# CC834/Heterogeneous-OpenCL-Image-Processing-Engine

Hardware: AMD Instinct MI355X
Metric: images_per_sec (higher is better)
Workload: dtype u8

## Files before the change

heterogeneous-opencl-image-processing-engine_amd/__init__.py:

```python
from __future__ import annotations

import ctypes as C
import os
import re
import subprocess

PKG_DIR = os.path.dirname(os.path.abspath(__file__))
ROOT = os.path.dirname(PKG_DIR)
CSRC = os.path.join(PKG_DIR, "csrc")
APPS = os.path.join(PKG_DIR, "apps")
LIB_PATH = os.path.join(PKG_DIR, "libmi_blur.so")
HEADER = os.path.join(ROOT, "include", "mi_blur.h")
HIPCC = os.environ.get("HIPCC", "/opt/rocm/bin/hipcc")
os.environ.setdefault("HIP_FORCE_DEV_KERNARG", "0")
ARCH = "gfx950"

DEVICE_CPU = -1
VARIANT_AUTO, VARIANT_GENERIC, VARIANT_TILED, VARIANT_STREAM, VARIANT_DIRECT = 0, 1, 2, 3, 4
OK, ERR_INVALID, ERR_NO_DEVICE, ERR_NOMEM, ERR_STATE, ERR_UNSUPPORTED = 0, -1, -2, -3, -4, -5
UNIQUE_ID_BYTES = 128
SEP_MAX_RADIUS = 16
MEDIAN_MAX_RADIUS = 7
MORPH_MAX_RADIUS = 16
MORPH_ERODE, MORPH_DILATE, MORPH_GRADIENT = 0, 1, 2
# ... 431 lines not shown
        "mi_blur_cpu_run_warp": (i, [u8p, u8p, i, i, i, i, C.POINTER(Warp), i]),
        "mi_blur_ctx_set_warp": (i, [vp, C.POINTER(Warp)]),
        "mi_blur_warp_perspective_coord": (i, [C.POINTER(WarpPerspective), i, i, C.POINTER(C.c_int64), C.POINTER(C.c_int64), C.POINTER(i), C.POINTER(i)]),
        "mi_blur_warp_perspective_quad": (i, [C.POINTER(C.c_double), C.POINTER(C.c_double), C.POINTER(C.c_double)]),
        "mi_blur_warp_perspective_set_matrix": (i, [C.POINTER(WarpPerspective), C.POINTER(C.c_double), i]),
        "mi_blur_enqueue_warp_perspective": (i, [u8p, u8p, i, i, i, i, C.POINTER(WarpPerspective), vp]),
        "mi_blur_cpu_run_warp_perspective": (i, [u8p, u8p, i, i, i, i, C.POINTER(WarpPerspective), i]),
        "mi_blur_ctx_set_warp_perspective": (i, [vp, C.POINTER(WarpPerspective)]),
        "mi_blur_remap_coord": (i, [C.POINTER(Remap), i, i, C.c_int32, C.c_int32, C.POINTER(i), C.POINTER(i), C.POINTER(i), C.POINTER(i)]),
        "mi_blur_remap_from_float": (i, [vp, vp, C.c_size_t, vp]),
        "mi_blur_remap_undistort": (i, [C.POINTER(C.c_double), C.POINTER(C.c_double), C.POINTER(C.c_double), i, i, vp]),
        "mi_blur_remap_plan": (i, [vp, i, i, i, C.POINTER(Remap), C.POINTER(RemapTiles)]),
        "mi_blur_enqueue_remap": (i, [u8p, u8p, i, i, i, i, C.POINTER(Remap), vp, vp]),
        "mi_blur_cpu_run_remap": (i, [u8p, u8p, i, i, i, i, C.POINTER(Remap), vp, i]),
        "mi_blur_ctx_set_remap": (i, [vp, C.POINTER(Remap), vp]),
        "mi_blur_conv_preset": (i, [i, C.POINTER(Conv)]),
        "mi_blur_enqueue_conv": (i, [u8p, u8p, i, i, i, i, C.POINTER(Conv), vp]),
        "mi_blur_enqueue_conv_band": (i, [u8p, u8p, i, i, i, i, i, C.POINTER(Conv), vp]),
        "mi_blur_cpu_run_conv": (i, [u8p, u8p, i, i, i, i, C.POINTER(Conv), i]),
        "mi_blur_ctx_set_conv": (i, [vp, C.POINTER(Conv)]),
        "mi_blur_fill_synthetic": (None, [u8p, i, i, i, i, i, i]),
        "mi_blur_fnv1a64": (C.c_uint64, [u8p, C.c_size_t]),
        "mi_blur_debug_zc_trace": (i, [vp, C.POINTER(C.c_uint64), i, C.POINTER(i), C.POINTER(C.c_uint)]),
        "mi_blur_debug_xcd_times": (i, [C.POINTER(C.c_uint64), C.POINTER(C.c_uint64), i]),
        "mi_blur_debug_xcd_raw": (i, [C.POINTER(C.c_uint64), C.c_size_t, C.c_size_t]),
        "mi_blur_a1_partition": (None, [i, i, C.c_float, C.POINTER(i), C.POINTER(i)]),
        "mi_blur_shard_range": (None, [C.c_longlong, i, i, C.POINTER(C.c_longlong), C.POINTER(C.c_longlong)]),
        "mi_blur_a2_split": (None, [i, C.c_float, i, C.POINTER(A2Geometry)]),
        "mi_blur_band_of": (None, [i, i, i, i, C.POINTER(Band)]),
        "mi_blur_comm_unique_id": (i, [vp]),
        "mi_blur_comm_init_rank": (i, [C.POINTER(vp), i, i, vp]),
        "mi_blur_comm_init_all": (i, [C.POINTER(vp), i, C.POINTER(i)]),
        "mi_blur_comm_init_p2p": (i, [C.POINTER(vp), i, C.POINTER(i)]),
        "mi_blur_comm_init_pull": (i, [C.POINTER(vp), i, C.POINTER(i)]),
        "mi_blur_comm_destroy": (None, [vp]),
        "mi_blur_comm_info": (i, [vp, C.POINTER(i), C.POINTER(i), C.POINTER(i)]),
        "mi_blur_halo_exchange": (i, [vp, u8p, i, i, i, i, vp]),
        "mi_blur_peer_export": (i, [vp, vp, C.POINTER(C.c_uint64)]),
        "mi_blur_peer_open": (i, [vp, C.c_uint64, C.POINTER(vp)]),
        "mi_blur_peer_close": (i, [vp, C.c_uint64]),
        "mi_blur_halo_pull": (i, [u8p, u8p, u8p, i, i, i, i, vp]),
        "mi_blur_enqueue_band_peer": (i, [u8p, u8p, i, i, i, i, i, i, u8p, u8p, vp]),
        "mi_blur_halo_exchange_all": (i, [C.POINTER(vp), i, C.POINTER(vp), i, i, C.POINTER(i), i, C.POINTER(vp)]),
    }
    for name, (res, args) in sig.items():
        fn = getattr(L, name)
        fn.restype, fn.argtypes = res, args
# ... 1069 lines not shown
```

heterogeneous-opencl-image-processing-engine_amd/csrc/blur_kernels.hip:

```cpp
#include "kernel_common.h"

#include <math.h>
#include <stdlib.h>
#include <string.h>
#include <mutex>
#include <algorithm>

namespace mi_blur {

__device__ __forceinline__ u16x2 as_pk(uint32_t x) { return __builtin_bit_cast(u16x2, x); }
__device__ __forceinline__ uint32_t as_u32(u16x2 x) { return __builtin_bit_cast(uint32_t, x); }

constexpr uint32_t EVEN_MASK = 0x00ff00ffu;
__device__ __forceinline__ uint32_t even_of(uint32_t x) { return x & EVEN_MASK; }
__device__ __forceinline__ uint32_t odd_of(uint32_t x) { return __builtin_amdgcn_perm(0u, x, 0x0c030c01u); }
__device__ __forceinline__ uint32_t mad6(uint32_t c, uint32_t t) { return as_u32(as_pk(c) * (unsigned short)6 + as_pk(t)); }

constexpr uint32_t sel_left(int C, int q)
{
    uint32_t s = 0;
    for (int j = 0; j < 4; j++) {
        int p = -4 * q + j;
        int idx = ((p % C) + C) % C;
        s |= (uint32_t)idx << (8 * j);
// ... 123 lines not shown
    }
    uint32_t Ew[8], Ow[8];
#pragma unroll
    for (int j = 0; j < 8; j++) { Ew[j] = even_of(w[j]); Ow[j] = odd_of(w[j]); }
    h[0] = hsum<C, R, 0, 0>(Ew, Ow); h[1] = hsum<C, R, 0, 1>(Ew, Ow);
    h[2] = hsum<C, R, 0, 2>(Ew, Ow); h[3] = hsum<C, R, 0, 3>(Ew, Ow);
    h[4] = hsum<C, R, 1, 0>(Ew, Ow); h[5] = hsum<C, R, 1, 1>(Ew, Ow);
    h[6] = hsum<C, R, 1, 2>(Ew, Ow); h[7] = hsum<C, R, 1, 3>(Ew, Ow);
}

struct TiledParams {
    const uint8_t *in;
    uint8_t *out;
    long long in_stride, out_stride;
    int pitch, cpr;
    int H, y0, y1;
    int ncols, nstrips;
    int TH, ntiles_y, ngroups;
    unsigned nblocks;
    int xcd;
    int debug_copy;
    unsigned long long *xcd_times;
    int tail;
};

struct __attribute__((packed, aligned(1))) Unaligned16 { u32x4 v; };
struct __attribute__((packed, aligned(1))) Unaligned8 { u32x2 v; };
struct __attribute__((packed, aligned(1))) Unaligned4 { uint32_t v; };
struct __attribute__((packed, aligned(1))) Unaligned2 { uint16_t v; };

__device__ __forceinline__ void store16_write_through(uint8_t *q, u32x4 v);
__device__ __forceinline__ void store_chunk_ragged_wt(uint8_t *q, u32x4 v, int n);
template <bool WT = false>
__device__ __forceinline__ void store_chunk_ragged(uint8_t *q, u32x4 v, int n)
{
    if constexpr (WT) { store_chunk_ragged_wt(q, v, n); return; }
    if (n >= 16) { reinterpret_cast<Unaligned16 *>(q)->v = v; return; }
    if (n & 8) { u32x2 t; t.x = v.x; t.y = v.y; reinterpret_cast<Unaligned8 *>(q)->v = t; q += 8; v.x = v.z; v.y = v.w; }
    if (n & 4) { reinterpret_cast<Unaligned4 *>(q)->v = v.x; q += 4; v.x = v.y; }
    if (n & 2) { reinterpret_cast<Unaligned2 *>(q)->v = (uint16_t)v.x; q += 2; v.x >>= 16; }
    if (n & 1) *q = (uint8_t)v.x;
}

__device__ __forceinline__ void store16_write_through(uint8_t *q, u32x4 v)
{
    asm volatile("global_store_dwordx4 %0, %1, off sc1\n\ts_nop 1" ::"v"(q), "v"(v) : "memory");
}

__device__ __forceinline__ void store_chunk_ragged_wt(uint8_t *q, u32x4 v, int n)
{
    if (n >= 16) { store16_write_through(q, v); return; }
    if (n & 8) {
        u32x2 t; t.x = v.x; t.y = v.y;
        asm volatile("global_store_dwordx2 %0, %1, off sc1" ::"v"(q), "v"(t) : "memory");
        q += 8; v.x = v.z; v.y = v.w;
    }
    if (n & 4) { asm volatile("global_store_dword %0, %1, off sc1" ::"v"(q), "v"(v.x) : "memory"); q += 4; v.x = v.y; }
    if (n & 2) { asm volatile("global_store_short %0, %1, off sc1" ::"v"(q), "v"(v.x) : "memory"); q += 2; v.x >>= 16; }
    if (n & 1) asm volatile("global_store_byte %0, %1, off sc1" ::"v"(q), "v"(v.x) : "memory");
}

struct NoHook { __device__ __forceinline__ void operator()() const {} };

template <int C, int R, int RPG, bool DMA, bool SHFL, bool RAG, bool WT = false, int X = rowpass_default<R>, typename Hook = NoHook>
__device__ __forceinline__ void tiled_tile(const TiledParams &p, unsigned L, Hook after_staging = Hook{})
{
    extern __shared__ __attribute__((aligned(16))) uint8_t lds[];
    const int t = threadIdx.x, NT = blockDim.x;
    const int strip = (int)(L % (unsigned)p.nstrips);
    const unsigned t2 = L / (unsigned)p.nstrips;
    const int ty = (int)(t2 % (unsigned)p.ntiles_y);
    const int img = (int)(t2 / (unsigned)p.ntiles_y);

    const int ty0 = p.y0 + ty * p.TH;
    const int rows_out = min(p.TH, p.y1 - ty0);
    const int x0c = strip * p.ncols;
    const int nc = min(p.ncols, p.cpr - x0c);
    const int cpr2 = nc + 2;
    const int nrows = rows_out + 2 * R;
    const uint8_t *img_in = p.in + (long long)img * p.in_stride;

    {
        const int lane = t & 63, wv = t >> 6, nwaves = NT >> 6;
        const int rpi = 64 / cpr2;
        const int lr = lane / cpr2, cc = lane - lr * cpr2;
        const bool dead_halo = (cc == 0 && x0c == 0) || (cc == cpr2 - 1 && x0c + nc == p.cpr);
        const bool act = lr < rpi && !dead_halo;
        const unsigned col_off = (unsigned)min(max(x0c + cc - 1, 0), p.cpr - 1) * 16u;
        for (int u = wv; u * rpi < nrows; u += nwaves) {
            const int row = u * rpi + lr;
            if (act && row < nrows) {
                const int sr = min(max(ty0 - R + row, 0), p.H - 1);
                const uint8_t *g = img_in + ((unsigned)sr * (unsigned)p.pitch + col_off);
                if constexpr (RAG) {
                    const uint8_t *rowp = img_in + (size_t)sr * (size_t)p.pitch;
                    uint8_t *dst = lds + (size_t)(u * rpi * cpr2 + lane) * 16u;
                    if (x0c + cc - 1 == p.cpr - 1) {
                        const u32x4 v = reinterpret_cast<const Unaligned16 *>(rowp + p.pitch - 16)->v;
                        reinterpret_cast<Unaligned16 *>(dst - (16 - p.tail))->v = v;
                        const int len = (16 - p.tail) + (cc == cpr2 - 1 ? 0 : 8);
                        uint8_t *pd = dst + p.tail;
                        const uint32_t fill[6] = {clamp_right<C, 0>(v.z, v.w), clamp_right<C, 1>(v.z, v.w), clamp_right<C, 2>(v.z, v.w),
                                                  clamp_right<C, 3>(v.z, v.w), clamp_right<C, 4>(v.z, v.w), clamp_right<C, 5>(v.z, v.w)};
#pragma unroll
                        for (int q = 0; q < 6; q++) {
                            if (4 * q + 4 <= len) reinterpret_cast<Unaligned4 *>(pd + 4 * q)->v = fill[q];
                            else if (4 * q < len)
                                for (int b = 0; b < len - 4 * q; b++) pd[4 * q + b] = (uint8_t)(fill[q] >> (8 * b));
                        }
                    } else if constexpr (DMA) {
                        uint8_t *base = lds + (size_t)(u * rpi * cpr2) * 16u;
                        __builtin_amdgcn_global_load_lds(
// ... 55 lines not shown
            if constexpr (R == 1) {
                const uint32_t se = (((hw[(r + 1) % WIN][i] << 1) + hw[r % WIN][i]) + hw[(r + 2) % WIN][i]) << 4;
                const uint32_t so = (((hw[(r + 1) % WIN][4 + i] << 1) + hw[r % WIN][4 + i]) + hw[(r + 2) % WIN][4 + i]) << 4;
                o[i] = __builtin_amdgcn_perm(so, se, 0x07030501u);
            } else {
                const uint32_t se = mad6(hw[(r + 2) % WIN][i],
                                         ((hw[(r + 1) % WIN][i] + hw[(r + 3) % WIN][i]) << 2) +
                                             (hw[r % WIN][i] + hw[(r + 4) % WIN][i]));
                const uint32_t so = mad6(hw[(r + 2) % WIN][4 + i],
                                         ((hw[(r + 1) % WIN][4 + i] + hw[(r + 3) % WIN][4 + i]) << 2) +
                                             (hw[r % WIN][4 + i] + hw[(r + 4) % WIN][4 + i]));
                o[i] = __builtin_amdgcn_perm(so, se, 0x07030501u);
            }
        }
        if (r0 + r < rows_out) {
            u32x4 v; v.x = o[0]; v.y = o[1]; v.z = o[2]; v.w = o[3];
            if constexpr (RAG) store_chunk_ragged<WT>(op + (size_t)r * (size_t)p.pitch, v, (x0c + col) == p.cpr - 1 ? p.tail : 16);
            else if constexpr (WT) store16_write_through(op + (size_t)r * (size_t)p.pitch, v);
            else *reinterpret_cast<u32x4 *>(op + (size_t)r * (size_t)p.pitch) = v;
        }
    }
}

constexpr unsigned XCD_DEBUG_SLOTS = 1u << 20;
__device__ __forceinline__ void xcd_time_mark(unsigned long long *t, unsigned long long t0)
{
    if (threadIdx.x == 0 && blockIdx.x < XCD_DEBUG_SLOTS) {
        unsigned id;
        asm volatile("s_getreg_b32 %0, hwreg(HW_REG_XCC_ID)" : "=s"(id));
        t[2u * blockIdx.x] = ((unsigned long long)__builtin_amdgcn_s_memrealtime() << 4) | (id & 7u);
        t[2u * blockIdx.x + 1] = t0;
    }
}

template <int C, int R, int RPG, bool DMA, bool SHFL = false, bool RAG = false>
__global__ __launch_bounds__(256) void blur_tiled_kernel(const TiledParams p)
{
    const unsigned long long t0 = p.xcd_times ? __builtin_amdgcn_s_memrealtime() : 0ull;
    tiled_tile<C, R, RPG, DMA, SHFL, RAG>(p, xcd_map(blockIdx.x, p.nblocks, p.xcd));
    if (p.xcd_times) xcd_time_mark(p.xcd_times, t0);
}

template <int C, int R, int RPG>
__global__ __launch_bounds__(256) void blur_tiled_loop_kernel(const TiledParams p)
{
    for (unsigned L = blockIdx.x; L < p.nblocks; L += gridDim.x) {
// ... 98 lines not shown
        const unsigned want = min(tiles_per_batch, total_blocks - first) * per_block;
        unsigned v = 0;
        for (unsigned k = lane; k < kcount; k += 64u) v += __hip_atomic_load(&count[kcount * n + k], __ATOMIC_RELAXED, __HIP_MEMORY_SCOPE_AGENT);
        v += __shfl_xor(v, 1); v += __shfl_xor(v, 2); v += __shfl_xor(v, 4); v += __shfl_xor(v, 8); v += __shfl_xor(v, 16); v += __shfl_xor(v, 32);
        v = __builtin_amdgcn_readfirstlane(v);
        if ((int)(v - want) >= 0) {
            n++;
            continue;
        }
        if (lane == 0) {
            const unsigned long long cur = ((unsigned long long)pass_seq << 32) | n;
            if (__hip_atomic_load(host_word, __ATOMIC_RELAXED, __HIP_MEMORY_SCOPE_SYSTEM) != cur)
                __hip_atomic_store(host_word, cur, __ATOMIC_RELEASE, __HIP_MEMORY_SCOPE_SYSTEM);
        }
        if (wall_clock64() - t0 > ZC_HARD_TICKS) return;
        __builtin_amdgcn_s_sleep(2);
    }
    if (lane == 0) __hip_atomic_store(host_word, ((unsigned long long)pass_seq << 32) | n, __ATOMIC_RELEASE, __HIP_MEMORY_SCOPE_SYSTEM);
}

static_assert(sizeof(TiledParams) <= ZC_PARAM_WORDS * 4 && sizeof(TiledParams) % 4 == 0, "TiledParams must fit a ZcBatch");
static_assert(sizeof(ZcBatch) / 4 <= 64, "the poller copies a descriptor with one wave-instruction");

template <int C, int R, int RPG, bool RAG>
__global__ __launch_bounds__(256) void blur_server_kernel(ZcHostCtl *ctl, ZcDevCtl *dev, unsigned seq, unsigned budget, unsigned idle_ticks,
                                                          unsigned long long *trace, int fixed_share)
{
    const unsigned NW = gridDim.x - 1;
    const unsigned first = dev->next[seq & 1u];

    if (blockIdx.x == NW) {
        const unsigned lane = threadIdx.x;
        if (lane >= 64) return;
        __shared__ unsigned s_ntiles[ZC_RING];
        unsigned g = dev->gnext[seq & 1u];
        if (lane == 0) {
            __hip_atomic_store(&dev->ticket, g, __ATOMIC_RELAXED, __HIP_MEMORY_SCOPE_AGENT);
            __hip_atomic_store(&dev->start_seq, seq + 1u, __ATOMIC_RELEASE, __HIP_MEMORY_SCOPE_AGENT);
        }
        unsigned k = first, c = first;
        const unsigned limit = first + budget;
        bool stopping = false;
        unsigned long long t_idle = wall_clock64();
        for (;;) {
            if (!stopping) {
                unsigned tail = 0;
                if (lane == 0) tail = __hip_atomic_load(&ctl->tail, __ATOMIC_ACQUIRE, __HIP_MEMORY_SCOPE_SYSTEM);
                tail = __builtin_amdgcn_readfirstlane(tail);
                const unsigned target = (int)(tail - limit) > 0 ? limit : tail;
                const bool progressed = (int)(target - k) > 0;
// ... 75 lines not shown
        }
        s_ctl[0] = ok;
    }
    __syncthreads();
    if (!s_ctl[0]) return;
    __syncthreads();
    union { TiledParams p; unsigned words[sizeof(TiledParams) / 4]; } u;
    unsigned k = first, have = 0u, tile_first = 0u, n_tiles = 0u;
    unsigned pending = ~0u;
    auto count_pending = [&]() {
        if (pending != ~0u && threadIdx.x == 0) {
            __builtin_amdgcn_fence(__ATOMIC_RELEASE, "");
            __hip_atomic_fetch_add(&dev->tiles_done[pending], 1u, __ATOMIC_RELEASE, __HIP_MEMORY_SCOPE_AGENT);
        }
        pending = ~0u;
    };
    auto flush_pending = [&]() {
        if (pending != ~0u) {
            asm volatile("s_waitcnt vmcnt(0)" ::: "memory");
            __syncthreads();
            count_pending();
        }
    };
    if (threadIdx.x == 0)
        s_ctl[1] = fixed_share ? dev->gnext[seq & 1u] + w : __hip_atomic_fetch_add(&dev->ticket, 1u, __ATOMIC_RELAXED, __HIP_MEMORY_SCOPE_AGENT);
    __syncthreads();
    unsigned t = s_ctl[1];
    unsigned long long *tr = nullptr;
    for (unsigned it = 0;; it++) {
        for (;;) {
            if (!have) {
                auto look = [&]() -> unsigned {
                    const unsigned a = __hip_atomic_load(&dev->avail, __ATOMIC_ACQUIRE, __HIP_MEMORY_SCOPE_AGENT);
                    if ((int)(a - k) > 0) return 1u;
                    if (__hip_atomic_load(&dev->stop_seq, __ATOMIC_ACQUIRE, __HIP_MEMORY_SCOPE_AGENT) == seq + 1u &&
                        (int)(__hip_atomic_load(&dev->stop_at, __ATOMIC_RELAXED, __HIP_MEMORY_SCOPE_AGENT) - k) <= 0) return 0u;
                    return 2u;
                };
                if (threadIdx.x == 0) s_ctl[0] = look();
                __syncthreads();
                unsigned go = s_ctl[0];
                __syncthreads();
                if (go != 1u) {
                    flush_pending();
                    if (go == 2u) {
                        if (threadIdx.x == 0) {
                            unsigned g2;
                            const unsigned long long t_w = wall_clock64();
                            while ((g2 = look()) == 2u) {
                                if (wall_clock64() - t_w > ZC_HARD_TICKS) { g2 = 0u; __hip_atomic_store(&ctl->error, 3u, __ATOMIC_RELEASE, __HIP_MEMORY_SCOPE_SYSTEM); break; }
// ... 4 lines not shown
                        __syncthreads();
                        go = s_ctl[0];
                        __syncthreads();
                    }
                    if (!go) return;
                }
                if (threadIdx.x < sizeof(ZcBatch) / 4)
                    s_words[threadIdx.x] = __hip_atomic_load(reinterpret_cast<unsigned *>(&dev->batch[k % ZC_RING]) + threadIdx.x, __ATOMIC_RELAXED,
                                                             __HIP_MEMORY_SCOPE_AGENT);
                __syncthreads();
#pragma unroll
                for (unsigned i = 0; i < sizeof(TiledParams) / 4; i++) u.words[i] = __builtin_amdgcn_readfirstlane(s_words[i]);
                tile_first = __builtin_amdgcn_readfirstlane(s_words[ZC_PARAM_WORDS]);
                n_tiles = __builtin_amdgcn_readfirstlane(s_words[ZC_PARAM_WORDS + 1]);
                have = 1u;
                __builtin_amdgcn_fence(__ATOMIC_ACQUIRE, "");
                __syncthreads();
            }
            if ((int)(t - (tile_first + n_tiles)) >= 0) { k++; have = 0u; continue; }
            break;
        }
        tr = (trace && k < ZC_TRACE_BATCHES && threadIdx.x == 0) ? trace + ((size_t)k * NW + w) * 5u : nullptr;
        if (tr) { if (tr[0] == 0) tr[0] = wall_clock64(); tr[1] += 1; }
        if (threadIdx.x == 0)
            s_ctl[2u + (it & 1u)] = fixed_share ? t + NW : __hip_atomic_fetch_add(&dev->ticket, 1u, __ATOMIC_RELAXED, __HIP_MEMORY_SCOPE_AGENT);
        const unsigned long long t_a = trace ? wall_clock64() : 0ull;
        tiled_tile<C, R, RPG, true, false, RAG, false, rowpass_default<R>>(u.p, t - tile_first, count_pending);
        pending = k % ZC_RING;
        __syncthreads();
        if (tr) { tr[2] += wall_clock64() - t_a; tr[3] = wall_clock64(); }
        t = s_ctl[2u + (it & 1u)];
    }
}

constexpr int STREAM_P = 6;
constexpr int STREAM_D = 8;
constexpr int STREAM_ROWB = 32 + 64 * 16;

struct StreamParams {
    const uint8_t *in;
    uint8_t *out;
    long long in_stride, out_stride;
    long long total;
    long long total_images;
    int pitch, cpr;
    int H, y0, y1;
    int BH, nbands;
    unsigned nblocks;
    int xcd;
    int updown;
};

struct StreamLane { unsigned col, band; long long img; };
__device__ __forceinline__ StreamLane stream_decode(unsigned f, const StreamParams &p)
// ... 431 lines not shown
            f.nextra = ntail + (unsigned)((long long)ntail * std::max(10, tun.fused_tail_blocks) / 100);
            g_last_kernel = "blur_fused_tail_kernel";
            const dim3 tgrid(f.nstatic + f.nextra);
            if (fused->gate && tun.fused_overlap > 0 && !ragged) {
                const long long ahead = nblocks * tun.fused_overlap / 1000;
                f.gate = fused->gate; f.gate_seq = fused->seq;
                f.gate_block = (unsigned)std::min<long long>(std::max<long long>(nblocks - ahead, 0), (long long)tgrid.x - 1);
            }
            if (p.xcd_times && tgrid.x <= 65536u) p.xcd_times += 2ull * 65536ull * (fused->seq & 15u);
            return dispatch<1, 2>(R, [&](auto Rc) { return launch_fused_r<Rc>(d, p, f, tgrid, block, lds, rpg, ragged); });
        }
        if (ragged) {
            if (!fused->tail_ctr) return MI_BLUR_ERR_UNSUPPORTED;
            f.tail_ctr = fused->tail_ctr; f.ntail = 0; f.nstatic = (unsigned)nblocks; f.nextra = 0;
            g_last_kernel = "blur_fused_tail_kernel";
        }
        return dispatch<1, 2>(R, [&](auto Rc) { return launch_fused_r<Rc>(d, p, f, grid, block, lds, rpg, ragged); });
    }
    return dispatch<1, 2>(R, [&](auto Rc) {
        return launch_tiled_r<Rc>(d, p, grid, block, lds, rpg, tun.stage_dma != 0, ragged, tun.row_shuffle != 0, tun.experiment);
    });
}

int zc_fill_batch(const LaunchDesc &d, ZcGeometry *geo, ZcBatch *b, unsigned *n_tiles)
{
    if (!geo || !b || !d.in || !d.out || d.n_images <= 0) return MI_BLUR_ERR_INVALID;
    Tunables tun = tunables();
    const bool aligned = tiled_eligible(d.in, d.out, d.width, d.channels) && !(d.in_stride % 16) && !(d.out_stride % 16);
    const long long pitch_b = (long long)d.width * d.channels;
    const bool dense = (!d.in_stride || d.in_stride == pitch_b * d.band_rows) && (!d.out_stride || d.out_stride == pitch_b * (d.y1 - d.y0));
    const bool ragged = !aligned && tun.ragged && ragged_eligible(d.width, d.channels) && dense;
    if (!aligned && !ragged) return MI_BLUR_ERR_UNSUPPORTED;
    tun.debug_copy = 0; tun.debug_xcd_times = 0; tun.xcd_remap = 0;
    TiledParams p{};
    unsigned threads = 0;
    size_t lds = 0;
    const int rpg = tiled_geometry(d, tun, ragged, false, 4, p, &threads, &lds);
    if (rpg < 0) return rpg;
    if (geo->threads == 0) { geo->threads = threads; geo->lds = lds; geo->rpg = rpg; geo->channels = d.channels; geo->radius = d.filter->radius; geo->ragged = ragged ? 1 : 0; }
    else if (geo->threads != threads || geo->lds != lds || geo->rpg != rpg || geo->channels != d.channels || geo->radius != d.filter->radius ||
             geo->ragged != (ragged ? 1 : 0))
        return MI_BLUR_ERR_UNSUPPORTED;
    memset(b->params, 0, sizeof b->params);
    memcpy(b->params, &p, sizeof p);
    if (n_tiles) *n_tiles = p.nblocks;
    return MI_BLUR_OK;
}

int zc_launch_server(const ZcGeometry &geo, ZcHostCtl *ctl, ZcDevCtl *dev, unsigned seq, unsigned n_workers, unsigned budget,
                     unsigned idle_ticks, hipStream_t stream, unsigned long long *trace, int fixed_share)
{
    if (!ctl || !dev || n_workers == 0 || geo.threads == 0 || geo.rpg != 4) return MI_BLUR_ERR_INVALID;
    g_last_kernel = "blur_server_kernel";
    const dim3 grid(n_workers + 1), block(geo.threads);
    return dispatch<0, 1>(geo.ragged, [&](auto RAG) {
        return dispatch<1, 2, 3, 4>(geo.channels, [&](auto C) {
            return dispatch<1, 2>(geo.radius, [&](auto R) {
                return do_launch(blur_server_kernel<C, R, 4, RAG != 0>, grid, block, geo.lds, stream, ctl, dev, seq, budget, idle_ticks, trace, fixed_share);
            });
        });
    });
}

int launch_fused_watch(const unsigned *count, unsigned n_batches, unsigned tiles_per_batch, unsigned total_blocks, unsigned per_block,
                       unsigned long long *host_word, unsigned pass_seq, hipStream_t stream, unsigned counters_per_batch)
{
    if (!count || !host_word || n_batches == 0 || tiles_per_batch == 0 || counters_per_batch < 8 || (counters_per_batch & (counters_per_batch - 1))) return MI_BLUR_ERR_INVALID;
    return do_launch(fused_watch_kernel, dim3(1), dim3(64), 0, stream, count, n_batches, tiles_per_batch, total_blocks, per_block, host_word, pass_seq, counters_per_batch);
}

int launch_fused_gate(const unsigned *gate, unsigned want, hipStream_t stream)
{
    if (!gate) return MI_BLUR_ERR_INVALID;
    return do_launch(fused_gate_kernel, dim3(1), dim3(64), 0, stream, gate, want);
}

int launch_fused(const LaunchDesc &d, const FusedDesc &f)
{
    if (!d.in || !d.out || d.in == d.out || (!f.count && !f.geometry_only) || f.batch_images <= 0) return MI_BLUR_ERR_INVALID;
    if (!d.filter || d.filter->kind != FilterKind::BOX) return MI_BLUR_ERR_INVALID;
    if (d.width <= 0 || d.band_rows <= 0 || d.n_images <= 0 || (d.filter->radius != 1 && d.filter->radius != 2)) return MI_BLUR_ERR_INVALID;
    if (d.y0 != 0 || d.y1 != d.band_rows || d.in_stride || d.out_stride) return MI_BLUR_ERR_INVALID;
// ... 155 lines not shown
```

heterogeneous-opencl-image-processing-engine_amd/csrc/blur_launch.h:

```cpp
#pragma once
#include <hip/hip_runtime.h>
#include <stdint.h>

#include "filter.h"

namespace mi_blur {

struct LaunchDesc {
    const Filter *filter;
    const uint8_t *in;
    uint8_t *out;
    int width, band_rows, channels;
    int n_images;
    int y0, y1;
    long long in_stride, out_stride;
    int concurrent;
    int max_blocks;
    int variant;
    const uint8_t *halo_top, *halo_bottom;
    hipStream_t stream;
    hipEvent_t start, stop;
};

int launch(const LaunchDesc &d);
// ... 55 lines not shown
    unsigned pad[6];
};
struct ZcHostCtl {
    unsigned tail;
    unsigned quit;
    unsigned servers_done;
    unsigned error;
    unsigned pad0[12];
    unsigned done[ZC_RING];
    unsigned long long t_begin[ZC_RING], t_end[ZC_RING];
    ZcBatch batch[ZC_RING];
};
struct ZcDevCtl {
    unsigned next[2];
    unsigned gnext[2];
    unsigned start_seq;
    unsigned avail;
    unsigned stop_seq, stop_at, stop_tile;
    unsigned ticket;
    unsigned pad[6];
    unsigned tiles_done[ZC_RING];
    ZcBatch batch[ZC_RING];
};
struct ZcGeometry { unsigned threads; size_t lds; int rpg; int channels, radius, ragged; };
int zc_fill_batch(const LaunchDesc &d, ZcGeometry *geo, ZcBatch *b, unsigned *n_tiles);
int zc_launch_server(const ZcGeometry &geo, ZcHostCtl *ctl, ZcDevCtl *dev, unsigned seq, unsigned n_workers, unsigned budget,
                     unsigned idle_ticks, hipStream_t stream, unsigned long long *trace = nullptr, int fixed_share = 0);

const char *last_kernel();

bool tiled_eligible(const void *in, const void *out, int width, int channels);

struct Tunables {
    int stage_dma; int rpg; int xcd_remap; int debug_copy; int row_shuffle; int prefer_stream; int stream_bh; int zero_copy; int ragged;
    int fused_release;
    int experiment;
    int xcd_run;
    int zero_copy_streams;
    int zero_copy_blocks;
    int stream_updown;
    int prefer_direct;
    int direct_bh;
    int debug_xcd_times;
    int fused_window;
    int fused_tail;
    int fused_adds_per_word;
    int fused_tail_blocks;
    int fused_overlap;
    int zero_copy_server;
    int zero_copy_server_min_kb;
    int staged_server;
    int zero_copy_workers;
    int zero_copy_idle_us;
    int zero_copy_budget;
    int zero_copy_tickets;
    int resident_place_trials;
    int zero_copy_spin;
    int zero_copy_trace;
    int zero_copy_debug_base;
    int zero_copy_events;
    int integral_band;
    int box_bytes;
    int dist_band;
    int dist_chunk_log2;
};
enum class KnobKind { FLAG, RANGE, ONE_OF };
struct Knob { const char *key; int Tunables::*field; KnobKind kind; int lo, hi, def; const char *env; };
constexpr int knob_bits(int a, int b, int c, int d) { return 1 << a | 1 << b | 1 << c | 1 << d; }
static constexpr Knob KNOBS[] = {
    {"stage_dma", &Tunables::stage_dma, KnobKind::FLAG, 0, 1, 1, "MI_BLUR_STAGE"},
    {"rows_per_thread", &Tunables::rpg, KnobKind::ONE_OF, knob_bits(0, 4, 8, 16), 0, 0, "MI_BLUR_RPG"},
    {"xcd_remap", &Tunables::xcd_remap, KnobKind::FLAG, 0, 1, 1, "MI_BLUR_XCD"},
    {"debug_copy", &Tunables::debug_copy, KnobKind::FLAG, 0, 1, 0, nullptr},
    {"row_shuffle", &Tunables::row_shuffle, KnobKind::FLAG, 0, 1, 0, nullptr},
    {"prefer_stream", &Tunables::prefer_stream, KnobKind::FLAG, 0, 1, 0, nullptr},
    {"zero_copy", &Tunables::zero_copy, KnobKind::FLAG, 0, 1, 1, nullptr},
    {"ragged_tiled", &Tunables::ragged, KnobKind::FLAG, 0, 1, 1, nullptr},
    {"stream_band_rows", &Tunables::stream_bh, KnobKind::RANGE, 0, 4096, 0, nullptr},
    {"fused_release", &Tunables::fused_release, KnobKind::FLAG, 0, 1, 0, nullptr},
    {"experiment", &Tunables::experiment, KnobKind::FLAG, 0, 1, 0, nullptr},
    {"stream_updown", &Tunables::stream_updown, KnobKind::FLAG, 0, 1, 1, nullptr},
    {"zero_copy_streams", &Tunables::zero_copy_streams, KnobKind::RANGE, 1, 8, 4, nullptr},
    {"zero_copy_blocks", &Tunables::zero_copy_blocks, KnobKind::RANGE, 0, 1 << 20, 24, nullptr},
    {"prefer_direct", &Tunables::prefer_direct, KnobKind::RANGE, 0, 2, 1, "MI_BLUR_DIRECT"},
    {"direct_bh", &Tunables::direct_bh, KnobKind::ONE_OF, knob_bits(4, 8, 12, 16), 0, 8, nullptr},
    {"fused_adds_per_word", &Tunables::fused_adds_per_word, KnobKind::RANGE, 4, 4096, 32, nullptr},
    {"fused_tail_blocks", &Tunables::fused_tail_blocks, KnobKind::RANGE, 10, 800, 25, nullptr},
    {"fused_tail", &Tunables::fused_tail, KnobKind::RANGE, 0, 500, 30, "MI_BLUR_FUSED_TAIL"},
    {"fused_overlap", &Tunables::fused_overlap, KnobKind::RANGE, 0, 500, 30, "MI_BLUR_FUSED_OVERLAP"},
    {"fused_window", &Tunables::fused_window, KnobKind::RANGE, 1, 4096, 8, nullptr},
    {"debug_xcd_times", &Tunables::debug_xcd_times, KnobKind::FLAG, 0, 1, 0, nullptr},
    {"zero_copy_events", &Tunables::zero_copy_events, KnobKind::FLAG, 0, 1, 1, nullptr},
    {"zero_copy_server", &Tunables::zero_copy_server, KnobKind::FLAG, 0, 1, 1, nullptr},
    {"staged_server", &Tunables::staged_server, KnobKind::FLAG, 0, 1, 1, "MI_BLUR_STAGED_SERVER"},
    {"zero_copy_server_min_kb", &Tunables::zero_copy_server_min_kb, KnobKind::RANGE, 0, 1 << 20, 1280, nullptr},
    {"zero_copy_trace", &Tunables::zero_copy_trace, KnobKind::FLAG, 0, 1, 0, nullptr},
    {"zero_copy_tickets", &Tunables::zero_copy_tickets, KnobKind::FLAG, 0, 1, 1, nullptr},
    {"zero_copy_spin", &Tunables::zero_copy_spin, KnobKind::FLAG, 0, 1, 0, nullptr},
    {"zero_copy_debug_base", &Tunables::zero_copy_debug_base, KnobKind::RANGE, 0, 1 << 20, 0, nullptr},
    {"resident_place_trials", &Tunables::resident_place_trials, KnobKind::RANGE, 0, 8, 4, "MI_BLUR_PLACE_TRIALS"},
    {"zero_copy_workers", &Tunables::zero_copy_workers, KnobKind::RANGE, 1, 2048, 48, nullptr},
    {"zero_copy_idle_us", &Tunables::zero_copy_idle_us, KnobKind::RANGE, 10, 100000, 300, nullptr},
    {"zero_copy_budget", &Tunables::zero_copy_budget, KnobKind::RANGE, 1, 1 << 20, 256, nullptr},
    {"xcd_run", &Tunables::xcd_run, KnobKind::RANGE, 0, 1 << 20, 0, nullptr},
    {"integral_band", &Tunables::integral_band, KnobKind::RANGE, 1, 256, 16, nullptr},
    {"box_bytes", &Tunables::box_bytes, KnobKind::ONE_OF, knob_bits(4, 16, 4, 16), 0, 4, nullptr},
    {"dist_band", &Tunables::dist_band, KnobKind::RANGE, 1, 256, 32, nullptr},
    {"dist_chunk_log2", &Tunables::dist_chunk_log2, KnobKind::RANGE, 3, 5, 4, nullptr},
};
static inline bool knob_set(const Knob &k, Tunables &t, int value)
{
    switch (k.kind) {
    case KnobKind::FLAG: t.*k.field = value != 0; return true;
    case KnobKind::RANGE: if (value < k.lo || value > k.hi) return false; break;
    case KnobKind::ONE_OF: if (value < 0 || value > 30 || !((k.lo >> value) & 1)) return false; break;
    }
    t.*k.field = value;
    return true;
}

// ... 7 lines not shown
```

heterogeneous-opencl-image-processing-engine_amd/csrc/mi_blur_api.cpp:

```cpp
#include "api_internal.h"
#include "blur_launch.h"
#include "cpu_device.h"

#include <sched.h>
#include <time.h>

#include <algorithm>
#include <chrono>
#include <climits>
#include <cmath>
#include <cstdio>
#include <cstdlib>
#include <cstring>
#include <mutex>
#include <new>
#include <deque>
#include <functional>
#include <condition_variable>
#include <thread>
#include <vector>

using namespace mi_blur;

__attribute__((constructor)) static void mi_blur_runtime_defaults() { setenv("HIP_FORCE_DEV_KERNARG", "0", 0); }
// ... 1206 lines not shown
            z->ctl->tail = B;
            for (unsigned i = 0; i < ZC_RING; i++) z->ctl->done[i] = B - ((B - i - 1u) % ZC_RING);
            z->head = B; z->tile_base = T;
        }
        if (e == hipSuccess) e = hipStreamSynchronize(z->stream);
        if (e != hipSuccess) {
            (void)hipGetLastError();
            if (z->stream) (void)hipStreamDestroy(z->stream);
            if (z->dev) (void)hipFree(z->dev);
            if (z->trace) (void)hipFree(z->trace);
            if (z->ctl) (void)hipHostFree(z->ctl);
            delete z;
            return MI_BLUR_ERR_HIP_BASE - (int)e;
        }
        z->fixed_share = tun.zero_copy_tickets ? 0 : 1;
        z->n_workers = (unsigned)tun.zero_copy_workers;
        z->budget = (unsigned)tun.zero_copy_budget;
        z->idle_ticks = (unsigned)tun.zero_copy_idle_us * 100u;
        c->zc = z;
    }
    ZcServer &z = *c->zc;
    ZcBatch b{};
    unsigned n_tiles = 0;
    int rc = zc_fill_batch(d, &z.geo, &b, &n_tiles);
    if (rc) return rc;
    if (n_tiles == 0 || z.n_workers / n_tiles + 2u * (unsigned)c->slots.size() + 2u > ZC_RING) return MI_BLUR_ERR_UNSUPPORTED;
    b.tile_first = z.tile_base;
    b.n_tiles = n_tiles;
    z.tile_base += n_tiles;
    const unsigned k = z.head;
    memcpy(&z.ctl->batch[k % ZC_RING], &b, sizeof b);
    __atomic_store_n(&z.ctl->tail, k + 1u, __ATOMIC_RELEASE);
    z.head = k + 1u;
    const unsigned stopped = __atomic_load_n(&z.ctl->servers_done, __ATOMIC_ACQUIRE);
    while (z.launched - stopped < 2u) {
        rc = zc_launch_server(z.geo, z.ctl_dev, z.dev, z.launched, z.n_workers, z.budget, z.idle_ticks, z.stream, z.trace, z.fixed_share);
        if (rc) return rc;
        z.launched++;
    }
    s.zc_server = true; s.zc_index = k;
    return MI_BLUR_OK;
}

static LaunchDesc ctx_launch(const mi_blur_ctx *c, const uint8_t *in, uint8_t *out, int band_rows, int n_images, int y0, int y1)
{
    LaunchDesc d{};
    d.filter = &c->filter;
    d.in = in; d.out = out; d.width = c->W; d.band_rows = band_rows; d.channels = c->C;
    d.n_images = n_images; d.y0 = y0; d.y1 = y1; d.variant = MI_BLUR_VARIANT_AUTO;
// ... 834 lines not shown
    HIP_TRY(hipDeviceSynchronize());
    HIP_TRY(hipMemcpy(out, d + 2 * first_slot, 16 * n_slots, hipMemcpyDeviceToHost));
    return MI_BLUR_OK;
}

extern "C" int mi_blur_debug_zc_trace(mi_blur_ctx *c, uint64_t *out, int max_batches, int *n_workers, unsigned *batches_published)
{
    if (!c || !out || max_batches <= 0) return MI_BLUR_ERR_INVALID;
    if (c->is_cpu() || !c->zc || !c->zc->trace) return MI_BLUR_ERR_STATE;
    ZcServer &z = *c->zc;
    HIP_TRY(hipSetDevice(c->device));
    const int nb = std::min<int>(max_batches, (int)ZC_TRACE_BATCHES);
    std::vector<unsigned long long> all;
    try { all.resize((size_t)ZC_TRACE_BATCHES * z.n_workers * 5u); } catch (...) { return MI_BLUR_ERR_NOMEM; }
    HIP_TRY(hipMemcpy(all.data(), z.trace, all.size() * sizeof(unsigned long long), hipMemcpyDeviceToHost));
    const int have = (int)std::min<unsigned>(z.head, (unsigned)nb);
    memcpy(out, all.data(), (size_t)have * z.n_workers * 5u * sizeof(unsigned long long));
    const int nb_out = have;
    if (n_workers) *n_workers = (int)z.n_workers;
    if (batches_published) *batches_published = z.head;
    return nb_out;
}

extern "C" uint64_t mi_blur_fnv1a64(const uint8_t *host, size_t n) { return fnv1a64(host, n); }

extern "C" void mi_blur_a1_partition(int mode, int batch_count, float gpu_ratio, int *n_cpu, int *n_gpu)
{
    int nc, ng;
    if (mode == 0) { ng = (int)(batch_count * gpu_ratio); nc = batch_count - ng; }
    else if (mode == 1) { nc = batch_count; ng = 0; }
    else { nc = 0; ng = batch_count; }
    if (n_cpu) *n_cpu = nc;
    if (n_gpu) *n_gpu = ng;
}

extern "C" void mi_blur_shard_range(long long n_units, int g, int G, long long *begin, long long *end)
{
    if (G <= 0) G = 1;
    if (begin) *begin = n_units * g / G;
    if (end) *end = n_units * (g + 1) / G;
}

extern "C" void mi_blur_a2_split(int height, float gpu_ratio, int halo, mi_blur_a2_geometry *g)
{
    if (!g) return;
    int split_row = (int)(height * (1.0f - gpu_ratio));
// ... 19 lines not shown
```

include/mi_blur.h:

```cpp
#ifndef MI_BLUR_H
#define MI_BLUR_H

#include <stddef.h>
#include <stdint.h>

#ifdef __cplusplus
extern "C" {
#endif

#define MI_BLUR_VERSION 1
#define MI_BLUR_DEVICE_CPU (-1)

typedef enum mi_blur_status {
    MI_BLUR_OK = 0,
    MI_BLUR_ERR_INVALID = -1,
    MI_BLUR_ERR_NO_DEVICE = -2,
    MI_BLUR_ERR_NOMEM = -3,
    MI_BLUR_ERR_STATE = -4,
    MI_BLUR_ERR_UNSUPPORTED = -5,
    MI_BLUR_ERR_HIP_BASE = -1000,
    MI_BLUR_ERR_RCCL_BASE = -2000
} mi_blur_status;

typedef enum mi_blur_variant {
// ... 420 lines not shown
} mi_blur_conv;

typedef enum mi_blur_conv_preset_id {
    MI_BLUR_CONV_SOBEL_X = 0, MI_BLUR_CONV_SOBEL_Y = 1, MI_BLUR_CONV_SOBEL_MAG = 2,
    MI_BLUR_CONV_SCHARR_X = 3, MI_BLUR_CONV_SCHARR_Y = 4, MI_BLUR_CONV_SCHARR_MAG = 5,
    MI_BLUR_CONV_LAPLACIAN4 = 6, MI_BLUR_CONV_LAPLACIAN8 = 7, MI_BLUR_CONV_SHARPEN = 8, MI_BLUR_CONV_EMBOSS = 9
} mi_blur_conv_preset_id;
int mi_blur_conv_preset(int preset, mi_blur_conv *k);

int mi_blur_enqueue_conv(const uint8_t *d_in, uint8_t *d_out, int width, int height, int channels, int n_images,
                         const mi_blur_conv *k, void *stream);
int mi_blur_enqueue_conv_band(const uint8_t *d_in, uint8_t *d_out, int width, int band_rows, int channels,
                              int out_row_begin, int out_row_end, const mi_blur_conv *k, void *stream);
int mi_blur_cpu_run_conv(const uint8_t *in, uint8_t *out, int width, int height, int channels, int n_images,
                         const mi_blur_conv *k, int n_threads);
int mi_blur_ctx_set_conv(mi_blur_ctx *ctx, const mi_blur_conv *k);

int mi_blur_debug_xcd_times(uint64_t end_ticks[8], uint64_t begin_ticks[8], int rearm);

int mi_blur_debug_xcd_raw(uint64_t *out, size_t first_slot, size_t n_slots);

int mi_blur_debug_zc_trace(mi_blur_ctx *ctx, uint64_t *out, int max_batches, int *n_workers, unsigned *batches_published);

void mi_blur_fill_synthetic(uint8_t *host, int width, int height, int channels,
                            int first_index, int n_images, int n_threads);
uint64_t mi_blur_fnv1a64(const uint8_t *host, size_t n);

void mi_blur_a1_partition(int mode, int batch_count, float gpu_ratio, int *n_cpu, int *n_gpu);
void mi_blur_shard_range(long long n_units, int g, int G, long long *begin, long long *end);

typedef struct mi_blur_a2_geometry {
    int split_row;
    int cpu_input_rows, cpu_output_rows;
    int gpu_input_rows, gpu_output_rows;
} mi_blur_a2_geometry;
void mi_blur_a2_split(int height, float gpu_ratio, int halo, mi_blur_a2_geometry *g);

typedef struct mi_blur_band {
    int row_begin, row_end;
    int halo_top, halo_bottom;
} mi_blur_band;
void mi_blur_band_of(int height, int radius, int g, int G, mi_blur_band *b);

typedef struct mi_blur_comm mi_blur_comm;
#define MI_BLUR_UNIQUE_ID_BYTES 128
int mi_blur_comm_unique_id(uint8_t id[MI_BLUR_UNIQUE_ID_BYTES]);
// ... 28 lines not shown
```

Before: 15.03 million.

## Claim tile runs in zero-copy server and reuse halo rows across vertical tiles

The persistent zero-copy blur server now grabs a run of consecutive tile tickets per atomic instead of one, and tiles are ordered column-major so a run walks down one strip. When consecutive tiles in the same batch are vertically adjacent, the 2R bottom halo rows already in LDS are copied to the top and not reloaded from global memory. This is meant to cut ticket atomics and redundant halo loads. The cost is coarser load balancing at batch tails, an extra LDS copy plus a barrier, and a wider ring-ahead check that can reject some configurations.

```diff
diff --git a/heterogeneous-opencl-image-processing-engine_amd/__init__.py b/heterogeneous-opencl-image-processing-engine_amd/__init__.py
--- a/heterogeneous-opencl-image-processing-engine_amd/__init__.py
+++ b/heterogeneous-opencl-image-processing-engine_amd/__init__.py
@@ -477,7 +477,9 @@
         "mi_blur_fill_synthetic": (None, [u8p, i, i, i, i, i, i]),
         "mi_blur_fnv1a64": (C.c_uint64, [u8p, C.c_size_t]),
         "mi_blur_debug_zc_trace": (i, [vp, C.POINTER(C.c_uint64), i, C.POINTER(i), C.POINTER(C.c_uint)]),
-        "mi_blur_debug_xcd_times": (i, [C.POINTER(C.c_uint64), C.POINTER(C.c_uint64), i]),
+        "mi_blur_debug_zc_plan": (i, [i, i, i, i, i, i, C.POINTER(i)]),
+        "mi_blur_debug_zc_tile": (i, [i, i, i, C.c_uint, C.POINTER(i)]),
+        "mi_blur_debug_xcd_times": (i,[C.POINTER(C.c_uint64), C.POINTER(C.c_uint64), i]),
         "mi_blur_debug_xcd_raw": (i, [C.POINTER(C.c_uint64), C.c_size_t, C.c_size_t]),
         "mi_blur_a1_partition": (None, [i, i, C.c_float, C.POINTER(i), C.POINTER(i)]),
         "mi_blur_shard_range": (None, [C.c_longlong, i, i, C.POINTER(C.c_longlong), C.POINTER(C.c_longlong)]),
diff --git a/heterogeneous-opencl-image-processing-engine_amd/csrc/blur_kernels.hip b/heterogeneous-opencl-image-processing-engine_amd/csrc/blur_kernels.hip
--- a/heterogeneous-opencl-image-processing-engine_amd/csrc/blur_kernels.hip
+++ b/heterogeneous-opencl-image-processing-engine_amd/csrc/blur_kernels.hip
@@ -169,7 +169,27 @@
     int debug_copy;
     unsigned long long *xcd_times;
     int tail;
+    int colmajor;
 };
+static_assert(sizeof(TiledParams) == 104, "colmajor sits in what was tail padding: no kernel's argument layout moves");
+
+struct TilePos { int strip, ty, img; };
+__host__ __device__ __forceinline__ TilePos tile_pos(unsigned L, int nstrips, int ntiles_y, bool colmajor)
+{
+    TilePos q;
+    if (colmajor) {
+        q.ty = (int)(L % (unsigned)ntiles_y);
+        const unsigned t2 = L / (unsigned)ntiles_y;
+        q.strip = (int)(t2 % (unsigned)nstrips);
+        q.img = (int)(t2 / (unsigned)nstrips);
+    } else {
+        q.strip = (int)(L % (unsigned)nstrips);
+        const unsigned t2 = L / (unsigned)nstrips;
+        q.ty = (int)(t2 % (unsigned)ntiles_y);
+        q.img = (int)(t2 / (unsigned)ntiles_y);
+    }
+    return q;
+}
 
 struct __attribute__((packed, aligned(1))) Unaligned16 { u32x4 v; };
 struct __attribute__((packed, aligned(1))) Unaligned8 { u32x2 v; };
@@ -209,15 +229,22 @@
 
 struct NoHook { __device__ __forceinline__ void operator()() const {} };
 
-template <int C, int R, int RPG, bool DMA, bool SHFL, bool RAG, bool WT = false, int X = rowpass_default<R>, typename Hook = NoHook>
-__device__ __forceinline__ void tiled_tile(const TiledParams &p, unsigned L, Hook after_staging = Hook{})
-{
+template <int C, int R, int RPG, bool DMA, bool SHFL, bool RAG, bool WT = false, int X = rowpass_default<R>, bool KEEP = false, typename Hook = NoHook>
+__device__ __forceinline__ void tiled_tile(const TiledParams &p, unsigned L, Hook after_staging = Hook{}, bool keep_top = false)
+{
+    static_assert(!KEEP || !RAG, "rows are kept between tiles in the aligned form only");
     extern __shared__ __attribute__((aligned(16))) uint8_t lds[];
     const int t = threadIdx.x, NT = blockDim.x;
-    const int strip = (int)(L % (unsigned)p.nstrips);
-    const unsigned t2 = L / (unsigned)p.nstrips;
-    const int ty = (int)(t2 % (unsigned)p.ntiles_y);
-    const int img = (int)(t2 / (unsigned)p.ntiles_y);
+    int strip, ty, img;
+    if constexpr (KEEP) {
+        const TilePos pos = tile_pos(L, p.nstrips, p.ntiles_y, p.colmajor != 0);
+        strip = pos.strip; ty = pos.ty; img = pos.img;
+    } else {
+        strip = (int)(L % (unsigned)p.nstrips);
+        const unsigned t2 = L / (unsigned)p.nstrips;
+        ty = (int)(t2 % (unsigned)p.ntiles_y);
+        img = (int)(t2 / (unsigned)p.ntiles_y);
+    }
 
     const int ty0 = p.y0 + ty * p.TH;
     const int rows_out = min(p.TH, p.y1 - ty0);
@@ -234,7 +261,9 @@
         const bool dead_halo = (cc == 0 && x0c == 0) || (cc == cpr2 - 1 && x0c + nc == p.cpr);
         const bool act = lr < rpi && !dead_halo;
         const unsigned col_off = (unsigned)min(max(x0c + cc - 1, 0), p.cpr - 1) * 16u;
-        for (int u = wv; u * rpi < nrows; u += nwaves) {
+        int u_first = wv;
+        if constexpr (KEEP) { if (keep_top) u_first += 2 * R / rpi; }
+        for (int u = u_first; u * rpi < nrows; u += nwaves) {
             const int row = u * rpi + lr;
             if (act && row < nrows) {
                 const int sr = min(max(ty0 - R + row, 0), p.H - 1);
@@ -336,6 +365,24 @@
     }
 }
 
+template <int R>
+__device__ __forceinline__ bool tiled_can_keep(const TiledParams &p, unsigned L)
+{
+    const TilePos pos = tile_pos(L, p.nstrips, p.ntiles_y, p.colmajor);
+    const int cpr2 = min(p.ncols, p.cpr - pos.strip * p.ncols) + 2;
+    return p.colmajor && pos.ty != 0 && (2 * R) % (64 / cpr2) == 0 && p.TH >= 2 * R;
+}
+template <int R>
+__device__ __forceinline__ void tiled_keep_rows(const TiledParams &p, unsigned L)
+{
+    extern __shared__ __attribute__((aligned(16))) uint8_t lds[];
+    const TilePos pos = tile_pos(L, p.nstrips, p.ntiles_y, p.colmajor);
+    const int cpr2 = min(p.ncols, p.cpr - pos.strip * p.ncols) + 2;
+    const int n = 2 * R * cpr2;
+    for (int i = threadIdx.x; i < n; i += blockDim.x)
+        *reinterpret_cast<uint4 *>(lds + (size_t)i * 16u) = *reinterpret_cast<const uint4 *>(lds + ((size_t)p.TH * cpr2 + i) * 16u);
+}
+
 constexpr unsigned XCD_DEBUG_SLOTS = 1u << 20;
 __device__ __forceinline__ void xcd_time_mark(unsigned long long *t, unsigned long long t0)
 {
@@ -480,10 +527,19 @@
 static_assert(sizeof(TiledParams) <= ZC_PARAM_WORDS * 4 && sizeof(TiledParams) % 4 == 0, "TiledParams must fit a ZcBatch");
 static_assert(sizeof(ZcBatch) / 4 <= 64, "the poller copies a descriptor with one wave-instruction");
 
+template <bool RUNS> struct ZcRunState {};
+template <> struct ZcRunState<true> {
+    unsigned t_end = 0u;
+    unsigned prev_t = 0u, prev_k = 0u;
+    bool have_prev = false;
+};
 template <int C, int R, int RPG, bool RAG>
 __global__ __launch_bounds__(256) void blur_server_kernel(ZcHostCtl *ctl, ZcDevCtl *dev, unsigned seq, unsigned budget, unsigned idle_ticks,
                                                           unsigned long long *trace, int fixed_share)
 {
+    constexpr bool RUNS = !RAG;
+    [[maybe_unused]] unsigned run = 1u;
+    if constexpr (RUNS) { run = max((unsigned)fixed_share >> 8, 1u); fixed_share &= 1; }
     const unsigned NW = gridDim.x - 1;
     const unsigned first = dev->next[seq & 1u];
 
@@ -605,10 +661,15 @@
             count_pending();
         }
     };
-    if (threadIdx.x == 0)
-        s_ctl[1] = fixed_share ? dev->gnext[seq & 1u] + w : __hip_atomic_fetch_add(&dev->ticket, 1u, __ATOMIC_RELAXED, __HIP_MEMORY_SCOPE_AGENT);
+    if (threadIdx.x == 0) {
+        if constexpr (RUNS) s_ctl[1] = fixed_share ? dev->gnext[seq & 1u] + w : __hip_atomic_fetch_add(&dev->ticket, run, __ATOMIC_RELAXED, __HIP_MEMORY_SCOPE_AGENT);
+        else s_ctl[1] = fixed_share ? dev->gnext[seq & 1u] + w : __hip_atomic_fetch_add(&dev->ticket, 1u, __ATOMIC_RELAXED, __HIP_MEMORY_SCOPE_AGENT);
+    }
     __syncthreads();
     unsigned t = s_ctl[1];
+    if constexpr (RUNS) t = __builtin_amdgcn_readfirstlane(t);
+    ZcRunState<RUNS> rs;
+    if constexpr (RUNS) rs.t_end = t + run;
     unsigned long long *tr = nullptr;
     for (unsigned it = 0;; it++) {
         for (;;) {
@@ -659,14 +720,34 @@
         }
         tr = (trace && k < ZC_TRACE_BATCHES && threadIdx.x == 0) ? trace + ((size_t)k * NW + w) * 5u : nullptr;
         if (tr) { if (tr[0] == 0) tr[0] = wall_clock64(); tr[1] += 1; }
-        if (threadIdx.x == 0)
-            s_ctl[2u + (it & 1u)] = fixed_share ? t + NW : __hip_atomic_fetch_add(&dev->ticket, 1u, __ATOMIC_RELAXED, __HIP_MEMORY_SCOPE_AGENT);
-        const unsigned long long t_a = trace ? wall_clock64() : 0ull;
-        tiled_tile<C, R, RPG, true, false, RAG, false, rowpass_default<R>>(u.p, t - tile_first, count_pending);
-        pending = k % ZC_RING;
-        __syncthreads();
-        if (tr) { tr[2] += wall_clock64() - t_a; tr[3] = wall_clock64(); }
-        t = s_ctl[2u + (it & 1u)];
+        if constexpr (RUNS) {
+            const bool last = t + 1u == rs.t_end;
+            if (threadIdx.x == 0 && last)
+                s_ctl[2u + (it & 1u)] = fixed_share ? t + NW : __hip_atomic_fetch_add(&dev->ticket, run, __ATOMIC_RELAXED, __HIP_MEMORY_SCOPE_AGENT);
+            const unsigned long long t_a = trace ? wall_clock64() : 0ull;
+            const unsigned L = t - tile_first;
+            const bool keep = run > 1u && rs.have_prev && t == rs.prev_t + 1u && k == rs.prev_k && tiled_can_keep<R>(u.p, L);
+            if (keep) {
+                tiled_keep_rows<R>(u.p, L);
+                __syncthreads();
+            }
+            tiled_tile<C, R, RPG, true, false, false, false, rowpass_default<R>, true>(u.p, L, count_pending, keep);
+            pending = k % ZC_RING;
+            __syncthreads();
+            if (tr) { tr[2] += wall_clock64() - t_a; tr[3] = wall_clock64(); tr[4] += keep ? 1u : 0u; }
+            rs.prev_t = t; rs.prev_k = k; rs.have_prev = true;
+            if (last) { t = __builtin_amdgcn_readfirstlane(s_ctl[2u + (it & 1u)]); rs.t_end = t + run; }
+            else t = t + 1u;
+        } else {
+            if (threadIdx.x == 0)
+                s_ctl[2u + (it & 1u)] = fixed_share ? t + NW : __hip_atomic_fetch_add(&dev->ticket, 1u, __ATOMIC_RELAXED, __HIP_MEMORY_SCOPE_AGENT);
+            const unsigned long long t_a = trace ? wall_clock64() : 0ull;
+            tiled_tile<C, R, RPG, true, false, RAG, false, rowpass_default<R>>(u.p, t - tile_first, count_pending);
+            pending = k % ZC_RING;
+            __syncthreads();
+            if (tr) { tr[2] += wall_clock64() - t_a; tr[3] = wall_clock64(); }
+            t = s_ctl[2u + (it & 1u)];
+        }
     }
 }
 
@@ -1144,7 +1225,21 @@
     });
 }
 
-int zc_fill_batch(const LaunchDesc &d, ZcGeometry *geo, ZcBatch *b, unsigned *n_tiles)
+int zc_pick_run(int option, int ntiles_y, unsigned n_tiles, unsigned n_workers)
+{
+    if (option >= 1) return std::min(option, (int)ZC_RUN_MAX);
+    if (ntiles_y <= 1 || n_workers == 0) return 1;
+    const unsigned per_draw = n_tiles / (ZC_RUN_DRAWS_PER_WORKER * n_workers);
+    return (int)std::max(1u, std::min({per_draw, (unsigned)ntiles_y, ZC_RUN_AUTO_MAX}));
+}
+
+void zc_tile_pos(unsigned L, int nstrips, int ntiles_y, int colmajor, int *strip, int *ty, int *img)
+{
+    const TilePos q = tile_pos(L, nstrips, ntiles_y, colmajor != 0);
+    *strip = q.strip; *ty = q.ty; *img = q.img;
+}
+
+int zc_fill_batch(const LaunchDesc &d, ZcGeometry *geo, ZcBatch *b, unsigned *n_tiles, unsigned n_workers, int *ntiles_y)
 {
     if (!geo || !b || !d.in || !d.out || d.n_images <= 0) return MI_BLUR_ERR_INVALID;
     Tunables tun = tunables();
@@ -1159,13 +1254,18 @@
     size_t lds = 0;
     const int rpg = tiled_geometry(d, tun, ragged, false, 4, p, &threads, &lds);
     if (rpg < 0) return rpg;
-    if (geo->threads == 0) { geo->threads = threads; geo->lds = lds; geo->rpg = rpg; geo->channels = d.channels; geo->radius = d.filter->radius; geo->ragged = ragged ? 1 : 0; }
+    if (geo->threads == 0) {
+        geo->threads = threads; geo->lds = lds; geo->rpg = rpg; geo->channels = d.channels; geo->radius = d.filter->radius; geo->ragged = ragged ? 1 : 0;
+        geo->run = (ragged || !tun.zero_copy_tickets) ? 1 : zc_pick_run(tun.zero_copy_run, p.ntiles_y, p.nblocks, n_workers);
+    }
     else if (geo->threads != threads || geo->lds != lds || geo->rpg != rpg || geo->channels != d.channels || geo->radius != d.filter->radius ||
              geo->ragged != (ragged ? 1 : 0))
         return MI_BLUR_ERR_UNSUPPORTED;
+    p.colmajor = geo->run > 1 ? 1 : 0;
     memset(b->params, 0, sizeof b->params);
     memcpy(b->params, &p, sizeof p);
     if (n_tiles) *n_tiles = p.nblocks;
+    if (ntiles_y) *ntiles_y = p.ntiles_y;
     return MI_BLUR_OK;
 }
 
@@ -1175,11 +1275,12 @@
     if (!ctl || !dev || n_workers == 0 || geo.threads == 0 || geo.rpg != 4) return MI_BLUR_ERR_INVALID;
     g_last_kernel = "blur_server_kernel";
     const dim3 grid(n_workers + 1), block(geo.threads);
-    return dispatch<0, 1>(geo.ragged, [&](auto RAG) {
-        return dispatch<1, 2, 3, 4>(geo.channels, [&](auto C) {
-            return dispatch<1, 2>(geo.radius, [&](auto R) {
-                return do_launch(blur_server_kernel<C, R, 4, RAG != 0>, grid, block, geo.lds, stream, ctl, dev, seq, budget, idle_ticks, trace, fixed_share);
-            });
+    const unsigned run = (fixed_share || geo.run < 1) ? 1u : (unsigned)geo.run;
+    return dispatch<1, 2, 3, 4>(geo.channels, [&](auto C) {
+        return dispatch<1, 2>(geo.radius, [&](auto R) {
+            if (geo.ragged) return do_launch(blur_server_kernel<C, R, 4, true>, grid, block, geo.lds, stream, ctl, dev, seq, budget, idle_ticks, trace, fixed_share);
+            return do_launch(blur_server_kernel<C, R, 4, false>, grid, block, geo.lds, stream, ctl, dev, seq, budget, idle_ticks, trace,
+                             (fixed_share ? 1 : 0) | (int)(run << 8));
         });
     });
 }
diff --git a/heterogeneous-opencl-image-processing-engine_amd/csrc/blur_launch.h b/heterogeneous-opencl-image-processing-engine_amd/csrc/blur_launch.h
--- a/heterogeneous-opencl-image-processing-engine_amd/csrc/blur_launch.h
+++ b/heterogeneous-opencl-image-processing-engine_amd/csrc/blur_launch.h
@@ -101,10 +101,13 @@
     unsigned tiles_done[ZC_RING];
     ZcBatch batch[ZC_RING];
 };
-struct ZcGeometry { unsigned threads; size_t lds; int rpg; int channels, radius, ragged; };
-int zc_fill_batch(const LaunchDesc &d, ZcGeometry *geo, ZcBatch *b, unsigned *n_tiles);
+struct ZcGeometry { unsigned threads; size_t lds; int rpg; int channels, radius, ragged; int run; };
+int zc_fill_batch(const LaunchDesc &d, ZcGeometry *geo, ZcBatch *b, unsigned *n_tiles, unsigned n_workers = 0, int *ntiles_y = nullptr);
 int zc_launch_server(const ZcGeometry &geo, ZcHostCtl *ctl, ZcDevCtl *dev, unsigned seq, unsigned n_workers, unsigned budget,
                      unsigned idle_ticks, hipStream_t stream, unsigned long long *trace = nullptr, int fixed_share = 0);
+constexpr unsigned ZC_RUN_MAX = 64, ZC_RUN_AUTO_MAX = 16, ZC_RUN_DRAWS_PER_WORKER = 1;
+int zc_pick_run(int option, int ntiles_y, unsigned n_tiles, unsigned n_workers);
+void zc_tile_pos(unsigned L, int nstrips, int ntiles_y, int colmajor, int *strip, int *ty, int *img);
 
 const char *last_kernel();
 
@@ -133,6 +136,7 @@
     int zero_copy_idle_us;
     int zero_copy_budget;
     int zero_copy_tickets;
+    int zero_copy_run;
     int resident_place_trials;
     int zero_copy_spin;
     int zero_copy_trace;
@@ -175,6 +179,7 @@
     {"zero_copy_server_min_kb", &Tunables::zero_copy_server_min_kb, KnobKind::RANGE, 0, 1 << 20, 1280, nullptr},
     {"zero_copy_trace", &Tunables::zero_copy_trace, KnobKind::FLAG, 0, 1, 0, nullptr},
     {"zero_copy_tickets", &Tunables::zero_copy_tickets, KnobKind::FLAG, 0, 1, 1, nullptr},
+    {"zero_copy_run", &Tunables::zero_copy_run, KnobKind::RANGE, 0, 64, 0, nullptr},
     {"zero_copy_spin", &Tunables::zero_copy_spin, KnobKind::FLAG, 0, 1, 0, nullptr},
     {"zero_copy_debug_base", &Tunables::zero_copy_debug_base, KnobKind::RANGE, 0, 1 << 20, 0, nullptr},
     {"resident_place_trials", &Tunables::resident_place_trials, KnobKind::RANGE, 0, 8, 4, "MI_BLUR_PLACE_TRIALS"},
diff --git a/heterogeneous-opencl-image-processing-engine_amd/csrc/mi_blur_api.cpp b/heterogeneous-opencl-image-processing-engine_amd/csrc/mi_blur_api.cpp
--- a/heterogeneous-opencl-image-processing-engine_amd/csrc/mi_blur_api.cpp
+++ b/heterogeneous-opencl-image-processing-engine_amd/csrc/mi_blur_api.cpp
@@ -1252,9 +1252,14 @@
     ZcServer &z = *c->zc;
     ZcBatch b{};
     unsigned n_tiles = 0;
-    int rc = zc_fill_batch(d, &z.geo, &b, &n_tiles);
+    const bool first_batch = z.geo.threads == 0;
+    int rc = zc_fill_batch(d, &z.geo, &b, &n_tiles, z.n_workers);
     if (rc) return rc;
-    if (n_tiles == 0 || z.n_workers / n_tiles + 2u * (unsigned)c->slots.size() + 2u > ZC_RING) return MI_BLUR_ERR_UNSUPPORTED;
+    const unsigned long long ahead = (unsigned long long)z.n_workers * (unsigned)std::max(1, z.geo.run);
+    if (n_tiles == 0 || ahead / n_tiles + 2u * (unsigned)c->slots.size() + 2u > ZC_RING) {
+        if (first_batch) z.geo = ZcGeometry{};
+        return MI_BLUR_ERR_UNSUPPORTED;
+    }
     b.tile_first = z.tile_base;
     b.n_tiles = n_tiles;
     z.tile_base += n_tiles;
@@ -2135,6 +2140,32 @@
     return nb_out;
 }
 
+extern "C" int mi_blur_debug_zc_plan(int width, int height, int channels, int radius, int n_images, int n_workers, int out[8])
+{
+    if (!out || width <= 0 || height <= 0 || channels <= 0 || n_images <= 0 || n_workers <= 0 || (radius != 1 && radius != 2)) return MI_BLUR_ERR_INVALID;
+    const Filter f = box_unchecked(radius);
+    alignas(16) static uint8_t in_tag[16], out_tag[16];
+    LaunchDesc d{};
+    d.filter = &f;
+    d.in = in_tag; d.out = out_tag; d.width = width; d.band_rows = height; d.channels = channels;
+    d.n_images = n_images; d.y0 = 0; d.y1 = height; d.variant = MI_BLUR_VARIANT_AUTO;
+    ZcGeometry geo{};
+    ZcBatch b{};
+    unsigned n_tiles = 0;
+    int ntiles_y = 0;
+    if (const int rc = zc_fill_batch(d, &geo, &b, &n_tiles, (unsigned)n_workers, &ntiles_y)) return rc;
+    out[0] = (int)(n_tiles / ((unsigned)ntiles_y * (unsigned)n_images)); out[1] = ntiles_y; out[2] = (int)n_tiles; out[3] = geo.ragged;
+    out[4] = geo.run; out[5] = geo.run > 1 ? 1 : 0; out[6] = (int)geo.threads; out[7] = (int)geo.lds;
+    return MI_BLUR_OK;
+}
+
+extern "C" int mi_blur_debug_zc_tile(int nstrips, int ntiles_y, int colmajor, unsigned tile, int out[3])
+{
+    if (!out || nstrips <= 0 || ntiles_y <= 0) return MI_BLUR_ERR_INVALID;
+    zc_tile_pos(tile, nstrips, ntiles_y, colmajor, &out[0], &out[1], &out[2]);
+    return MI_BLUR_OK;
+}
+
 extern "C" uint64_t mi_blur_fnv1a64(const uint8_t *host, size_t n) { return fnv1a64(host, n); }
 
 extern "C" void mi_blur_a1_partition(int mode, int batch_count, float gpu_ratio, int *n_cpu, int *n_gpu)
diff --git a/include/mi_blur.h b/include/mi_blur.h
--- a/include/mi_blur.h
+++ b/include/mi_blur.h
@@ -466,6 +466,9 @@
 
 int mi_blur_debug_zc_trace(mi_blur_ctx *ctx, uint64_t *out, int max_batches, int *n_workers, unsigned *batches_published);
 
+int mi_blur_debug_zc_plan(int width, int height, int channels, int radius, int n_images, int n_workers, int out[8]);
+int mi_blur_debug_zc_tile(int nstrips, int ntiles_y, int colmajor, unsigned tile, int out[3]);
+
 void mi_blur_fill_synthetic(uint8_t *host, int width, int height, int channels,
                             int first_index, int n_images, int n_threads);
 uint64_t mi_blur_fnv1a64(const uint8_t *host, size_t n);
```

Measured after the change: 15.02 million (median of 2 runs). No clear change (-0.0%).
